# microsoft/ANCE

Hardware: AMD Instinct MI355X
Metric: passages_encoded_per_sec (higher is better)
Workload: dtype f16 pair operands on the fp16 MFMA, f32 accumulate (fp32-grade: <= 2e-5 from the reference's fp32 forward); 1 GPU; MS MARCO passage 8841823 x 768-d, roberta-base rdot_nll FirstP seq_len=128, encode + brute-force IP top-200 (BASELINE configs[1]); encode_block_per_gpu=16384, query_block=32768, layers=12, parallelism=dp1 (corpus rows sharded, top-k all-to-all by query owner + merge)

## Files before the change

ance_amd/csrc/attention.h:

```cpp
#pragma once
#include "common.h"

namespace ance {

struct AttnArgs {
    const _Float16 *qk;
    const _Float16 *vt;
    _Float16 *ctx;
    const int4 *desc;
    int ld_qk, ld_vt, ld_ctx;
    int n_heads;
    int cls_only;
    int q_compact;
};

size_t attention_lds_bytes(int max_seq_len, int n_waves);
int launch_attention_split(const float *qkv, _Float16 *ctx_pair, const int4 *desc, int n_seq, int n_heads, int max_seq_len,
                           int cls_only, hipStream_t stream);
int launch_attention(const AttnArgs &args, int n_seq, int max_seq_len, hipStream_t stream);

}
```

ance_amd/csrc/attention.hip:

```cpp
#include <stdio.h>
#include <stdlib.h>
#include <type_traits>
#include <vector>

#include "common.h"
#include "attention.h"
#include "precise32.h"

namespace ance {
namespace {

constexpr int HD = 64;

__device__ __forceinline__ int kswz(int row, int chunk) { return chunk ^ ((row >> 1) & 7); }

__device__ __forceinline__ void wave_lds_sync() {
    __builtin_amdgcn_fence(__ATOMIC_SEQ_CST, "wavefront");
    __builtin_amdgcn_wave_barrier();
}

__device__ __forceinline__ void attend_qblock(const AttnArgs &A, const _Float16 *Ks, const _Float16 *Vs, const f16x8 (&qf)[4], int s,
                                              int h, int tok0, int T, int Tk, int vld, int qb0, int q_end, int g, int i,
                                              _Float16 *slab) {
    const int nkb = Tk >> 5;
// ... 92 lines not shown
    const int s = dsc.w;
    const int Tk = (T + 31) & ~31;
    const int vld = Tk + 4;
    _Float16 *Ks = reinterpret_cast<_Float16 *>(smem_f);
    _Float16 *Vs = Ks + (size_t)Tk * HD;

    const int tid = threadIdx.x;
    const int w = tid >> 6, l = tid & 63, g = l >> 5, i = l & 31;
    const int H = A.n_heads * HD;
    _Float16 *slab = Vs + (size_t)HD * vld + w * (32 * HD);

    const int q_end = A.cls_only ? 1 : T;
    f16x8 qf[4];
    auto q_row = [&](int r) { return A.q_compact ? (size_t)s : (size_t)(tok0 + min(r, T - 1)); };
    auto q_request = [&](int qb0) {
#pragma unroll
        for (int j = 0; j < 4; ++j) {
            const int row = j * 8 + (l >> 3);
            qf[j] = *reinterpret_cast<const f16x8 *>(A.qk + q_row(qb0 + row) * A.ld_qk + h * HD + (l & 7) * 8);
        }
    };
    auto q_to_fragments = [&]() {
#pragma unroll
        for (int j = 0; j < 4; ++j) {
            const int row = j * 8 + (l >> 3);
            *reinterpret_cast<f16x8 *>(slab + row * HD + kswz(row, l & 7) * 8) = qf[j];
        }
        wave_lds_sync();
#pragma unroll
        for (int sx = 0; sx < 4; ++sx) qf[sx] = *reinterpret_cast<const f16x8 *>(slab + i * HD + kswz(i, 4 * g + sx) * 8);
        wave_lds_sync();
    };
    if (w * 32 < q_end) q_request(w * 32);

    {
        const _Float16 *kbase = A.qk + (size_t)tok0 * A.ld_qk + H + h * HD + (tid & 7) * 8;
        const _Float16 *vbase = A.vt + (size_t)(h * HD) * A.ld_vt + vcol0;
        for (int base = 0; base < Tk; base += 32 * NW) {
            f16x8 kv[4], vv[4];
#pragma unroll
            for (int j = 0; j < 4; ++j) {
                const int row = base + j * (8 * NW) + (tid >> 3);
                const int ev = j * NT + tid, dd = ev / (4 * NW);
                const int key0 = base + (ev - dd * (4 * NW)) * 8;
                kv[j] = f16x8{0, 0, 0, 0, 0, 0, 0, 0};
                vv[j] = f16x8{0, 0, 0, 0, 0, 0, 0, 0};
                if (row < T) kv[j] = *reinterpret_cast<const f16x8 *>(kbase + (size_t)row * A.ld_qk);
                if (key0 < T) vv[j] = *reinterpret_cast<const f16x8 *>(vbase + (size_t)dd * A.ld_vt + key0);
            }
#pragma unroll
            for (int j = 0; j < 4; ++j) {
                const int row = base + j * (8 * NW) + (tid >> 3);
                const int ev = j * NT + tid, dd = ev / (4 * NW);
                const int key0 = base + (ev - dd * (4 * NW)) * 8;
                if (row < Tk) *reinterpret_cast<f16x8 *>(Ks + row * HD + kswz(row, tid & 7) * 8) = kv[j];
                if (key0 < Tk) {
                    if (key0 + 8 > T) {
#pragma unroll
                        for (int e = 0; e < 8; ++e)
                            if (key0 + e >= T) vv[j][e] = (_Float16)0.0f;
                    }
                    _Float16 *dst = Vs + dd * vld + key0;
                    *reinterpret_cast<f16x4 *>(dst) = f16x4{vv[j][0], vv[j][1], vv[j][2], vv[j][3]};
                    *reinterpret_cast<f16x4 *>(dst + 4) = f16x4{vv[j][4], vv[j][5], vv[j][6], vv[j][7]};
                }
            }
        }
    }
    if (w * 32 < q_end) q_to_fragments();
    __syncthreads();

    for (int qb0 = w * 32; qb0 < q_end; qb0 += 32 * NW) {
        if (qb0 != w * 32) {
            q_request(qb0);
            q_to_fragments();
        }
        attend_qblock(A, Ks, Vs, qf, s, h, tok0, T, Tk, vld, qb0, q_end, g, i, slab);
    }
}



constexpr int VS = HD;
__device__ __forceinline__ int vswz(int key, int d) { return d ^ (((key >> 1) & 1) << 5); }
typedef short s16x4_t __attribute__((ext_vector_type(4)));
typedef s16x4_t __attribute__((address_space(3))) lds_s16x4_t;
__device__ __forceinline__ f16x4 lds_read_tr16(const _Float16 *p) {
    const s16x4_t v = __builtin_amdgcn_ds_read_tr16_b64_v4i16((lds_s16x4_t *)(p));
    return __builtin_bit_cast(f16x4, v);
}

__device__ __forceinline__ void permlane32_swap(float &x, float &y) {
    asm volatile("s_nop 1\n\tv_permlane32_swap_b32 %0, %1\n\ts_nop 1" : "+v"(x), "+v"(y));
}

template <int NW>
__global__ void __launch_bounds__(64 * NW, 2) attention_split_kernel(const float *qkv, _Float16 *ctx_pair, const int4 *desc, int n_heads,
                                                                     int cls_only, int kchunk) {
    extern __shared__ __attribute__((aligned(16))) float smem_f[];
    const int u = blockIdx.x / n_heads;
    const int h = blockIdx.x - u * n_heads;
    const int4 dsc = desc[u];
    const int tok0 = dsc.x, T = dsc.y, s = dsc.w;
    const int Tk = (T + 31) & ~31;
    const int kc = Tk < kchunk ? Tk : kchunk;
    _Float16 *Kh = reinterpret_cast<_Float16 *>(smem_f);
    _Float16 *Kl = Kh + (size_t)kc * HD;
    _Float16 *Vh = Kl + (size_t)kc * HD;
    _Float16 *Vl = Vh + (size_t)kc * VS;
    const int tid = threadIdx.x;
    const int w = tid >> 6, l = tid & 63, g = l >> 5, i = l & 31;
    constexpr int NT = 64 * NW;
    const int ld = 3 * n_heads * HD;
    constexpr float SC = 2048.0f, SI = 1.0f / 2048.0f;
    auto stage = [&](int k0, auto unr_tag) {
        constexpr int UNR = decltype(unr_tag)::value;
        for (int e0 = tid; e0 < kc * 8; e0 += UNR * NT) {
            f32x4 kv[UNR][4];
#pragma unroll
            for (int it = 0; it < UNR; ++it) {
                const int e = e0 + it * NT;
                const int kl_ = e >> 3, ch = e & 7, key = k0 + kl_;
#pragma unroll
                for (int q = 0; q < 4; ++q) kv[it][q] = f32x4{0.f, 0.f, 0.f, 0.f};
                if (e < kc * 8 && key < T) {
                    const float *kp = qkv + (size_t)(tok0 + key) * ld + n_heads * HD + h * HD + ch * 8;
                    kv[it][0] = *reinterpret_cast<const f32x4 *>(kp);
                    kv[it][1] = *reinterpret_cast<const f32x4 *>(kp + 4);
                    kv[it][2] = *reinterpret_cast<const f32x4 *>(kp + n_heads * HD);
                    kv[it][3] = *reinterpret_cast<const f32x4 *>(kp + n_heads * HD + 4);
                }
            }
#pragma unroll
            for (int it = 0; it < UNR; ++it) {
                const int e = e0 + it * NT;
                if (e >= kc * 8) break;
                const int kl_ = e >> 3, ch = e & 7;
                const f32x4 k0v = kv[it][0], k1v = kv[it][1], v0 = kv[it][2], v1 = kv[it][3];
                const f16x4 a0 = cvt_f16x4_pinned(k0v), a1 = cvt_f16x4_pinned(k1v), b0 = cvt_f16x4_pinned(v0), b1 = cvt_f16x4_pinned(v1);
                f16x8 kh, kl;
#pragma unroll
                for (int j = 0; j < 4; ++j) {
                    kh[j] = a0[j]; kh[4 + j] = a1[j];
                    kl[j] = (_Float16)((k0v[j] - (float)a0[j]) * SC);
                    kl[4 + j] = (_Float16)((k1v[j] - (float)a1[j]) * SC);
                }
                *reinterpret_cast<f16x8 *>(Kh + kl_ * HD + kswz(kl_, ch) * 8) = kh;
                *reinterpret_cast<f16x8 *>(Kl + kl_ * HD + kswz(kl_, ch) * 8) = kl;
                f16x8 vh, vl;
#pragma unroll
                for (int j = 0; j < 4; ++j) {
                    vh[j] = b0[j]; vh[4 + j] = b1[j];
                    vl[j] = (_Float16)((v0[j] - (float)b0[j]) * SC);
                    vl[4 + j] = (_Float16)((v1[j] - (float)b1[j]) * SC);
                }
                *reinterpret_cast<f16x8 *>(Vh + kl_ * VS + vswz(kl_, ch * 8)) = vh;
                *reinterpret_cast<f16x8 *>(Vl + kl_ * VS + vswz(kl_, ch * 8)) = vl;
            }
        }
    };
    const bool single = Tk <= kc;
    const int q_end = cls_only ? 1 : T;
    const float qscale = 0.125f * 1.44269504088896340736f;
    for (int qp0 = 0; qp0 < q_end; qp0 += 32 * NW) {
        const int qb0 = qp0 + w * 32;
        const bool active = qb0 < q_end;
        f16x8 qh[4], ql[4];
        {
            const float *qp = qkv + (cls_only ? (size_t)s : (size_t)(tok0 + min(qb0 + i, T - 1))) * ld + h * HD + 32 * g;
            f32x4 xq[8];
#pragma unroll
            for (int sx = 0; sx < 8; ++sx) xq[sx] = *reinterpret_cast<const f32x4 *>(qp + sx * 4);
            if (single && qp0 == 0) {
                stage(0, std::integral_constant<int, 4>{});
                __syncthreads();
            }
#pragma unroll
            for (int sx = 0; sx < 4; ++sx) {
                f32x4 x0 = xq[2 * sx], x1 = xq[2 * sx + 1];
                x0 = x0 * qscale;
                x1 = x1 * qscale;
                const f16x4 a0 = cvt_f16x4_pinned(x0), a1 = cvt_f16x4_pinned(x1);
#pragma unroll
                for (int j = 0; j < 4; ++j) {
                    qh[sx][j] = a0[j]; qh[sx][4 + j] = a1[j];
                    ql[sx][j] = (_Float16)((x0[j] - (float)a0[j]) * SC);
                    ql[sx][4 + j] = (_Float16)((x1[j] - (float)a1[j]) * SC);
                }
            }
        }
        float m_run = -INFINITY, l_run = 0.0f;
        f32x16 om0 = {0}, om1 = {0}, oc0 = {0}, oc1 = {0};
        for (int k0 = 0; k0 < Tk; k0 += kc) {
            if (!single) {
                __syncthreads();
                stage(k0, std::integral_constant<int, 1>{});
                __syncthreads();
            }
            if (!active) continue;
            const int nkb = min(kc, Tk - k0) >> 5;
            for (int kb = 0; kb < nkb; ++kb) {
                const int krow = kb * 32 + i;
                const int ksw = (krow >> 1) & 7;
                f32x16 st = {0};
                f16x8 kfh[4];
#pragma unroll
                for (int sx = 0; sx < 4; ++sx) {
                    kfh[sx] = *reinterpret_cast<const f16x8 *>(Kh + krow * HD + (((4 * g + sx) ^ ksw) * 8));
                    const f16x8 kfl = *reinterpret_cast<const f16x8 *>(Kl + krow * HD + (((4 * g + sx) ^ ksw) * 8));
                    st = __builtin_amdgcn_mfma_f32_32x32x16_f16(kfh[sx], ql[sx], st, 0, 0, 0);
                    st = __builtin_amdgcn_mfma_f32_32x32x16_f16(kfl, qh[sx], st, 0, 0, 0);
                }
                st *= SI;
#pragma unroll
                for (int sx = 0; sx < 4; ++sx) st = __builtin_amdgcn_mfma_f32_32x32x16_f16(kfh[sx], qh[sx], st, 0, 0, 0);
                const int key_base = k0 + kb * 32 + 4 * g;
                float bm = -INFINITY;
#pragma unroll
                for (int r = 0; r < 16; ++r) {
                    const int key = key_base + (r & 3) + 8 * (r >> 2);
                    if (k0 + kb * 32 + 32 > T) st[r] = key < T ? st[r] : -INFINITY;
                    bm = fmaxf(bm, st[r]);
                }
                bm = fmaxf(bm, __shfl_xor(bm, 32));
                const float m_new = fmaxf(m_run, bm);
                const float alpha = __builtin_amdgcn_exp2f(m_run - m_new);
                float psum = 0.0f;
                float p[16];
#pragma unroll
                for (int r = 0; r < 16; ++r) {
                    p[r] = __builtin_amdgcn_exp2f(st[r] - m_new);
                    psum += p[r];
                }
                l_run = l_run * alpha + psum;
                m_run = m_new;
                om0 *= alpha; om1 *= alpha; oc0 *= alpha; oc1 *= alpha;
#pragma unroll
                for (int uu = 0; uu < 2; ++uu) {
                    const f16x4 h0 = cvt_f16x4_pinned(f32x4{p[8 * uu], p[8 * uu + 1], p[8 * uu + 2], p[8 * uu + 3]});
                    const f16x4 h1 = cvt_f16x4_pinned(f32x4{p[8 * uu + 4], p[8 * uu + 5], p[8 * uu + 6], p[8 * uu + 7]});
                    f16x8 ph, pl;
#pragma unroll
                    for (int j = 0; j < 4; ++j) {
                        ph[j] = h0[j]; ph[4 + j] = h1[j];
                        pl[j] = (_Float16)((p[8 * uu + j] - (float)h0[j]) * SC);
                        pl[4 + j] = (_Float16)((p[8 * uu + 4 + j] - (float)h1[j]) * SC);
                    }
                    const int kcol = kb * 32 + 16 * uu + 4 * g;
                    auto vfrag = [&](const _Float16 *V, int row) {
                        const int q = l & 15, key = kcol + (q >> 2);
                        const _Float16 *vp = V + key * VS + vswz(key, (row - i) + 16 * ((l >> 4) & 1) + 4 * (q & 3));
                        const f16x4 a = lds_read_tr16(vp), b = lds_read_tr16(vp + 8 * VS);
                        return f16x8{a[0], a[1], a[2], a[3], b[0], b[1], b[2], b[3]};
                    };
                    const f16x8 v0h = vfrag(Vh, i), v1h = vfrag(Vh, i + 32), v0l = vfrag(Vl, i), v1l = vfrag(Vl, i + 32);
                    oc0 = __builtin_amdgcn_mfma_f32_32x32x16_f16(v0h, pl, oc0, 0, 0, 0);
                    oc0 = __builtin_amdgcn_mfma_f32_32x32x16_f16(v0l, ph, oc0, 0, 0, 0);
                    oc1 = __builtin_amdgcn_mfma_f32_32x32x16_f16(v1h, pl, oc1, 0, 0, 0);
                    oc1 = __builtin_amdgcn_mfma_f32_32x32x16_f16(v1l, ph, oc1, 0, 0, 0);
                    om0 = __builtin_amdgcn_mfma_f32_32x32x16_f16(v0h, ph, om0, 0, 0, 0);
                    om1 = __builtin_amdgcn_mfma_f32_32x32x16_f16(v1h, ph, om1, 0, 0, 0);
                }
            }
        }
        if (!active) continue;
        const float l_tot = l_run + __shfl_xor(l_run, 32);
        const float inv = 1.0f / l_tot;
        {
            const bool store = qb0 + i < q_end;
            const size_t orow = cls_only ? (size_t)s : (size_t)(tok0 + min(qb0 + i, T - 1));
            _Float16 *orp = ctx_pair + orow * (size_t)(2 * n_heads * HD);
#pragma unroll
            for (int db = 0; db < 2; ++db) {
                const f32x16 &om = db == 0 ? om0 : om1;
                const f32x16 &oc = db == 0 ? oc0 : oc1;
#pragma unroll
                for (int k2 = 0; k2 < 2; ++k2) {
                    f32x4 va, vb;
#pragma unroll
                    for (int j = 0; j < 4; ++j) {
                        const float xa = __builtin_fmaf(oc[8 * k2 + j], SI, om[8 * k2 + j]) * inv;
                        const float xb = __builtin_fmaf(oc[8 * k2 + 4 + j], SI, om[8 * k2 + 4 + j]) * inv;
                        float sa = xa, sb = xb;
                        permlane32_swap(sa, sb);
                        va[j] = sa;
                        vb[j] = sb;
                    }
                    if (store) {
                        f16x4 ha, ra, hb, rb;
                        pair_split4(va, &ha, &ra);
                        pair_split4(vb, &hb, &rb);
                        const int n = h * HD + db * 32 + 16 * k2 + 8 * g;
                        *reinterpret_cast<f16x8 *>(orp + pair_hi_col(n, n_heads * HD)) = f16x8{ha[0], ha[1], ha[2], ha[3], hb[0], hb[1], hb[2], hb[3]};
                        *reinterpret_cast<f16x8 *>(orp + pair_lo_col(n, n_heads * HD)) = f16x8{ra[0], ra[1], ra[2], ra[3], rb[0], rb[1], rb[2], rb[3]};
                    }
                }
            }
        }
    }
}

}

size_t attention_split_lds_bytes(int max_seq_len) {
    const int Tk = (max_seq_len + 31) & ~31;
    return (size_t)2 * Tk * HD * 2 + (size_t)2 * Tk * VS * 2;
}

int launch_attention_split(const float *qkv, _Float16 *ctx_pair, const int4 *desc, int n_seq, int n_heads, int max_seq_len,
                           int cls_only, hipStream_t st) {
    if (n_seq <= 0) return ANCE_OK;
    const int Tk = (max_seq_len + 31) & ~31;
    const int kchunk = Tk <= 256 ? Tk : 256;
    const size_t lds = attention_split_lds_bytes(kchunk);
    int dev = 0;
    (void)hipGetDevice(&dev);
    static size_t attr_set[64] = {0};
    const bool tracked = dev >= 0 && dev < 64;
    if (!tracked || lds > __atomic_load_n(&attr_set[dev], __ATOMIC_ACQUIRE)) {
        if (hipFuncSetAttribute(reinterpret_cast<const void *>(attention_split_kernel<4>), hipFuncAttributeMaxDynamicSharedMemorySize,
                                (int)lds) != hipSuccess)
            return check_launch("attention_split attr");
        if (tracked) __atomic_store_n(&attr_set[dev], lds, __ATOMIC_RELEASE);
    }
    hipLaunchKernelGGL((attention_split_kernel<4>), dim3((unsigned)n_seq * n_heads), dim3(256), lds, st, qkv, ctx_pair, desc, n_heads,
                       cls_only, kchunk);
    return ANCE_OK;
}

size_t attention_lds_bytes(int max_seq_len, int n_waves) {
    const int Tk = (max_seq_len + 31) & ~31;
    return (size_t)Tk * HD * 2 + (size_t)HD * (Tk + 4) * 2 + (size_t)n_waves * 32 * HD * 2;
}

int launch_attention(const AttnArgs &A, int n_seq, int max_seq_len, hipStream_t st) {
    if (n_seq <= 0) return ANCE_OK;
    const size_t lds = attention_lds_bytes(max_seq_len, 4);
    if (lds > 160 * 1024) {
        set_last_error("attention: sequence too long for LDS");
        return ANCE_E_INVALID;
    }
    int dev = 0;
    (void)hipGetDevice(&dev);
    static size_t attr_set[64] = {0};
    const bool tracked = dev >= 0 && dev < 64;
    if (!tracked || lds > __atomic_load_n(&attr_set[dev], __ATOMIC_ACQUIRE)) {
        if (hipFuncSetAttribute(reinterpret_cast<const void *>(attention_kernel<4>),
                                hipFuncAttributeMaxDynamicSharedMemorySize, (int)lds) != hipSuccess)
            return check_launch("attention attr");
        if (tracked) __atomic_store_n(&attr_set[dev], lds, __ATOMIC_RELEASE);
    }
    hipLaunchKernelGGL((attention_kernel<4>), dim3((unsigned)n_seq * A.n_heads), dim3(256), lds, st, A);
    return ANCE_OK;
}

}

extern "C" int ance_debug_attention(const AnceAttnDebugArgs *a, void *stream) {
    using namespace ance;
    auto refuse = [](const char *why) {
        char buf[160];
        snprintf(buf, sizeof(buf), "ance_debug_attention: invalid argument (%s)", why);
        set_last_error(buf);
        return ANCE_E_INVALID;
    };
    if (!a) return refuse("null args");
    if (a->kind < 0 || a->kind > 2) return refuse("kind");
    if (a->n_heads != 12 && a->n_heads != 16) return refuse("n_heads");
    if (a->n_seq < 1 || a->n_seq > (1 << 20)) return refuse("n_seq");
    if (a->max_seq_len < 1 || a->max_seq_len > 512) return refuse("max_seq_len");
    if (!a->h_desc || !a->d_desc || !a->qk || !a->ctx || (a->kind == 0 && !a->vt)) return refuse("null pointer");
    const int64_t H = 64 * (int64_t)a->n_heads, n = a->n_seq;
    const int64_t desc_bytes = a->kind == 2 ? 4 * (n + 1) : 16 * n;
    if (a->d_desc_bytes < desc_bytes || (uintptr_t)a->d_desc % 16) return refuse("d_desc");
    if ((uintptr_t)a->qk % 16 || (uintptr_t)a->ctx % 16 || (a->kind == 0 && (uintptr_t)a->vt % 16)) return refuse("alignment");
    if (a->qk_rows < 1 || a->ctx_rows < 1) return refuse("rows");
    if (a->kind == 0) {
        if (a->ld_qk % 8 || a->ld_qk < 2 * H || a->ld_vt % 8 || a->ld_vt < 8 || a->ld_ctx % 8 || a->ld_ctx < H) return refuse("stride");
    } else {
        if (a->ld_qk != 3 * H || a->ld_ctx != (a->kind == 1 ? 2 * H : H)) return refuse("stride");
    }
    if (a->kind == 2 && (a->cls_only || a->q_compact)) return refuse("cls_only on kind 2");
    if (a->kind == 1 && a->q_compact != a->cls_only) return refuse("kind 1: q_compact != cls_only");
    if (a->kind == 0 && a->q_compact && !a->cls_only) return refuse("q_compact without cls_only");
    const int32_t *d = a->h_desc;
    if (a->kind == 2) {
        if (d[0] < 0) return refuse("tokens outside the allocation");
        for (int64_t s = 0; s < n; ++s) {
            const int64_t len = (int64_t)d[s + 1] - d[s];
            if (len < 1 || len > a->max_seq_len) return refuse("length");
        }
        if (d[n] > a->qk_rows || d[n] > a->ctx_rows) return refuse("tokens outside the allocation");
    } else {
        std::vector<char> seen((size_t)n, 0);
        const bool compact = a->cls_only && (a->q_compact || a->kind == 1);
        for (int64_t u = 0; u < n; ++u) {
            const int64_t tok0 = d[4 * u], len = d[4 * u + 1], vcol = d[4 * u + 2], s = d[4 * u + 3];
            if (len < 1 || len > a->max_seq_len) return refuse("length");
            if (s < 0 || s >= n || seen[(size_t)s]) return refuse("sequence index");
            seen[(size_t)s] = 1;
            if (tok0 < 0 || tok0 + len > a->qk_rows) return refuse("tokens outside the allocation");
            if (compact && s >= a->qk_rows) return refuse("Q row s past the allocation");
            if (a->cls_only ? s >= a->ctx_rows : tok0 + len > a->ctx_rows) return refuse("output row past the allocation");
            if (a->kind == 0 && (vcol < 0 || vcol % 8 || vcol + ((len + 7) & ~7) > a->ld_vt)) return refuse("V^T columns");
        }
    }
    hipStream_t st = (hipStream_t)stream;
    if (hipMemcpyAsync(a->d_desc, a->h_desc, (size_t)desc_bytes, hipMemcpyHostToDevice, st) != hipSuccess)
        return check_launch("ance_debug_attention: descriptors");
    int rc;
    if (a->kind == 0) {
        AttnArgs A;
        A.qk = (const _Float16 *)a->qk; A.vt = (const _Float16 *)a->vt; A.ctx = (_Float16 *)a->ctx; A.desc = (const int4 *)a->d_desc;
        A.ld_qk = a->ld_qk; A.ld_vt = a->ld_vt; A.ld_ctx = a->ld_ctx; A.n_heads = a->n_heads;
        A.cls_only = a->cls_only ? 1 : 0; A.q_compact = a->q_compact ? 1 : 0;
        rc = launch_attention(A, a->n_seq, a->max_seq_len, st);
    } else if (a->kind == 1) {
        rc = launch_attention_split((const float *)a->qk, (_Float16 *)a->ctx, (const int4 *)a->d_desc, a->n_seq, a->n_heads,
                                    a->max_seq_len, a->cls_only ? 1 : 0, st);
    } else {
        rc = launch_attention32((const float *)a->qk, (float *)a->ctx, (const int *)a->d_desc, a->n_seq, a->n_heads, st);
    }
    return rc ? rc : check_launch("ance_debug_attention");
}
```

ance_amd/csrc/encoder.hip:

```cpp
#include <stdlib.h>
#include <type_traits>
#include <vector>

#include "attention.h"
#include "common.h"
#include "encoder_kernels.h"
#include "encoder_plan.h"
#include "gemm_f16.h"
#include "precise32.h"

namespace ance {
namespace {

template <typename F>
auto with_hidden(int hidden, F &&f) {
    return hidden == 1024 ? f(std::integral_constant<int, 1024>()) : f(std::integral_constant<int, 768>());
}

constexpr int S_CAP_MAX = 8192;
constexpr int FETCH_CHUNK = 262144;
constexpr int MAX_LANES = 2;


bool precise_env() {
// ... 269 lines not shown
}

template <int H>
GemmArgs qk_args(const Rows<FORM_PLANES> &x, int M, float eps, const LayerW &W, int c0, int n, _Float16 *qk) {
    GemmArgs G = folded_args<H>(x, M, eps, W.wqk + (size_t)c0 * H, n, W.bqk + c0, W.cqk + c0);
    G.out16 = qk + c0; G.ldc = 2 * H;
    G.scale = 0.125f * 1.44269504088896340736f; G.scale_cols = c0 == 0 ? H : 0;
    return G;
}
template <int H>
GemmArgs qkv_args(const Rows<FORM_PAIR> &x, int M, float eps, const LayerW &W, int c0, int n, float *qkv, unsigned *faults) {
    GemmArgs G = folded_args<H>(x, M, eps, W.wqkv_s + (size_t)c0 * 2 * H, n, W.bqkv_s + c0, W.cqkv_s + c0, W.sc_s + 4, faults);
    G.out32 = qkv + c0; G.ldc = 3 * H;
    return G;
}

template <int H>
GemmArgs vt_args(const Rows<FORM_PLANES> &x, int Tpad, int T, float eps, const LayerW &W, _Float16 *vt, int ldvt, const int *col_map) {
    GemmArgs G = {};
    G.A = W.wv; G.lda = H; G.B = x.hi; G.tok_lo = x.lo; G.ldb = H; G.M = H; G.N = Tpad; G.K = H;
    G.bias = W.bv; G.csum = W.cv; G.part_in = x.part; G.ln_eps = eps;
    G.out16 = vt; G.ldc = ldvt; G.col_map = col_map; G.n_valid = T;
    return G;
}

template <int H, int FORM>
GemmArgs ffn1_args(const Rows<FORM> &xa, int M, float eps, const LayerW &W, int I, _Float16 *ffn, int n_split, unsigned *faults) {
    constexpr bool P = FORM == FORM_PAIR;
    GemmArgs G = folded_args<H>(xa, M, eps, P ? W.w1_s : W.w1, I, P ? W.b1_s : W.b1, P ? W.c1_s : W.c1, P ? W.sc_s + 6 : nullptr, faults);
    G.out16 = ffn; G.ldc = P ? 2 * I : I; G.n_split = n_split;
    return G;
}

template <int H, int FORM>
GemmArgs resln_args(const _Float16 *A, const _Float16 *B, int K, const float *bias, int M, const Rows<FORM> &res, const float *gamma,
                    const float *beta, float eps, const Rows<FORM> &out, const float *wscale_inv, unsigned *faults) {
    constexpr int w = FORM == FORM_PAIR ? 2 : 1;
    GemmArgs G = {};
    G.A = A; G.lda = w * K; G.B = B; G.ldb = w * K; G.M = M; G.N = H; G.K = K; G.bias = bias; G.ldc = w * H;
    G.res_gamma = gamma; G.res_beta = beta; G.part_in = res.part; G.ln_eps = eps; G.part_out = out.part;
    G.wscale_inv = wscale_inv; G.range_faults = faults;
    if constexpr (FORM == FORM_PAIR) { G.res_hi = res.xp; G.ldr = 2 * H; G.out16 = out.xp; }
    else { G.res_hi = res.hi; G.res_lo = res.lo; G.out16 = out.hi; G.out_lo = out.lo; }
    return G;
}

template <int H>
int forward_split(AnceEncoder *e, const AnceEncoder::Lane &LN, hipStream_t st, const MicroPlan &mb, float *out) {
    constexpr int HP = 2 * H;
    const AnceEncoderDesc &D = e->d;
    const AnceEncoder::Lane::Split &V = LN.sp;
    const int I = D.intermediate, S = mb.S, T = mb.T, Tpad = mb.Tpad;
    {
        ProfScope pe(PC_EMBED, st);
        hipLaunchKernelGGL((embed_kernel<H, FORM_PAIR>), dim3(Tpad / 4), dim3(256), 0, st, LN.tok_id, LN.tok_pos, Tpad, e->word,
                           e->pos, e->type0, D.vocab_size, D.max_position, V.xb, e->faults);
    }
    const bool cls_tail = e->cls_tail;
    const int S_pad = (int)align_up((size_t)S, 256);
    const Rows<FORM_PAIR> cls = V.cls(S_pad, H);
    const int n_split = (I / 256) % 2 == 0 ? 2 : 0;
    for (int li = 0; li < D.n_layers; ++li) {
        const LayerW &W = e->layers[li];
        const bool tail = cls_tail && li == D.n_layers - 1;
        const int Mrows = tail ? S_pad : Tpad;
        const double Mwork = tail ? (double)S : (double)T;
        const float eps_b = li == 0 ? D.ln_eps * (EMB_SCALE * EMB_SCALE) : D.ln_eps;
        const float *const gamma_b = li == 0 ? e->eln_w : e->layers[li - 1].ln2w, *const beta_b = li == 0 ? e->eln_b : e->layers[li - 1].ln2b;
        if (tail) {
            ProfScope ps(PC_LN, st);
            hipLaunchKernelGGL((gather_cls_kernel<H, FORM_PAIR>), dim3(S_pad / 4), dim3(256), 0, st, V.xb, LN.seq_off, S, S_pad, cls);
        }
        {
            ProfScope ps(PC_GEMM_QK, st, tail ? 2.0 * T * (2.0 * H) * H + 2.0 * S * (double)H * H : 2.0 * T * (3.0 * H) * H);
            const int c0 = tail ? H : 0;
            int rc = launch_gemm_f16(EPI_S_QKV, qkv_args<H>(V.xb, Tpad, eps_b, W, c0, 3 * H - c0, V.qkv, e->faults), st, H);
            if (tail && !rc) rc = launch_gemm_f16(EPI_S_QKV, qkv_args<H>(cls, S_pad, eps_b, W, 0, H, V.qkv, e->faults), st, H);
            if (rc) return rc;
        }
        {
            ProfScope ps(PC_ATTN, st);
            if (tail && S_pad > S)
                (void)hipMemsetAsync(V.ctx + (size_t)S * HP, 0, (size_t)(S_pad - S) * HP * sizeof(_Float16), st);
            if (int rc = launch_attention_split(V.qkv, V.ctx, LN.desc, S, D.n_heads, mb.maxlen, tail ? 1 : 0, st)) return rc;
        }
        if (ProfScope ps(PC_GEMM_OUT, st, 2.0 * Mwork * (double)H * H);
            int rc = launch_gemm_f16(EPI_S_RESLN, resln_args<H>(V.ctx, W.wo_s, H, W.bo, Mrows, tail ? cls : V.xb, gamma_b, beta_b, eps_b,
                                                                V.xa, W.sc_s + 5, e->faults), st, H))
            return rc;
        if (ProfScope ps(PC_GEMM_FFN1, st, 2.0 * Mwork * (double)I * H);
            int rc = launch_gemm_f16(EPI_S_GELU, ffn1_args<H>(V.xa, Mrows, D.ln_eps, W, I, V.ffn, n_split, e->faults), st, H))
            return rc;
        if (ProfScope ps(PC_GEMM_FFN2, st, 2.0 * Mwork * (double)I * H);
            int rc = launch_gemm_f16(EPI_S_RESLN, resln_args<H>(V.ffn, W.w2_s, I, W.b2, Mrows, V.xa, W.ln1w, W.ln1b, D.ln_eps, V.xb,
                                                                W.sc_s + 7, e->faults), st, H))
            return rc;
    }
    encoder_output<H>(e, LN, st, mb, out, V.xb, cls_tail ? 1 : 0);
    return ANCE_OK;
}

template <int H>
int forward_fp16(AnceEncoder *e, const AnceEncoder::Lane &LN, hipStream_t st, const MicroPlan &mb, float *out) {
    const AnceEncoderDesc &D = e->d;
    const AnceEncoder::Lane::Fp16 &V = LN.f16;
    const int I = D.intermediate, S = mb.S, T = mb.T, Tpad = mb.Tpad;
    {
        ProfScope pe(PC_EMBED, st);
        hipLaunchKernelGGL((embed_kernel<H, FORM_PLANES>), dim3(Tpad / 4), dim3(256), 0, st, LN.tok_id, LN.tok_pos, Tpad, e->word,
                           e->pos, e->type0, D.vocab_size, D.max_position, V.xb, (unsigned *)nullptr);
    }
    const bool cls_tail = e->cls_tail;
    const int S_pad = (int)align_up((size_t)S, 256);
    const Rows<FORM_PLANES> cls = V.cls(S_pad, H);
    const int n_split = (I / 256) % 2 == 0 ? 2 : 0;
    for (int li = 0; li < D.n_layers; ++li) {
        const LayerW &W = e->layers[li];
        const bool tail = cls_tail && li == D.n_layers - 1;
        const int Mrows = tail ? S_pad : Tpad;
        const double Mwork = tail ? (double)S : (double)T;
        const float *const gamma_b = li == 0 ? e->eln_w : e->layers[li - 1].ln2w, *const beta_b = li == 0 ? e->eln_b : e->layers[li - 1].ln2b;
        if (tail) {
            ProfScope ps(PC_LN, st);
            hipLaunchKernelGGL((gather_cls_kernel<H, FORM_PLANES>), dim3(S_pad / 4), dim3(256), 0, st, V.xb, LN.seq_off, S, S_pad, cls);
        }
        {
            ProfScope ps(PC_GEMM_QK, st, tail ? 2.0 * T * (double)H * H + 2.0 * S * (double)H * H : 2.0 * T * (2.0 * H) * H);
            const int c0 = tail ? H : 0;
            int rc = launch_gemm_f16(EPI_QK_F, qk_args<H>(V.xb, Tpad, D.ln_eps, W, c0, 2 * H - c0, V.qk), st, H);
            if (tail && !rc) rc = launch_gemm_f16(EPI_QK_F, qk_args<H>(cls, S_pad, D.ln_eps, W, 0, H, V.qk), st, H);
            if (rc) return rc;
        }
        if (ProfScope ps(PC_GEMM_VT, st, 2.0 * T * (double)H * H);
            int rc = launch_gemm_f16(EPI_VT_F, vt_args<H>(V.xb, Tpad, T, D.ln_eps, W, V.vt, mb.ldvt, LN.tok_vtcol), st, H))
            return rc;
        AttnArgs A;
        A.qk = V.qk; A.vt = V.vt; A.ctx = V.ctx; A.desc = LN.desc;
        A.ld_qk = 2 * H; A.ld_vt = mb.ldvt; A.ld_ctx = H; A.n_heads = D.n_heads; A.cls_only = tail ? 1 : 0; A.q_compact = tail ? 1 : 0;
        if (ProfScope ps(PC_ATTN, st, 0.0); int rc = launch_attention(A, S, mb.maxlen, st)) return rc;
        if (ProfScope ps(PC_GEMM_OUT, st, 2.0 * Mwork * (double)H * H);
            int rc = launch_gemm_f16(EPI_RESLN, resln_args<H>(V.ctx, W.wo, H, W.bo, Mrows, tail ? cls : V.xb, gamma_b, beta_b, D.ln_eps,
                                                              V.xa, nullptr, nullptr), st, H))
            return rc;
        if (ProfScope ps(PC_GEMM_FFN1, st, 2.0 * Mwork * (double)I * H);
            int rc = launch_gemm_f16(EPI_GELU_F, ffn1_args<H>(V.xa, Mrows, D.ln_eps, W, I, V.ffn, n_split, nullptr), st, H))
            return rc;
        if (ProfScope ps(PC_GEMM_FFN2, st, 2.0 * Mwork * (double)I * H);
            int rc = launch_gemm_f16(EPI_RESLN, resln_args<H>(V.ffn, W.w2, I, W.b2, Mrows, V.xa, W.ln1w, W.ln1b, D.ln_eps, V.xb,
                                                              nullptr, nullptr), st, H))
            return rc;
    }
    encoder_output<H>(e, LN, st, mb, out, V.xb, cls_tail ? 1 : 0);
    return ANCE_OK;
}

struct LaneFork {
    AnceEncoder *e;
    hipStream_t caller_st;
    bool forked = false;
    void fork() {
        (void)hipEventRecord(e->ev_fork, caller_st);
        for (int ln = 0; ln < e->n_lanes; ++ln) (void)hipStreamWaitEvent(e->side[ln], e->ev_fork, 0);
        forked = true;
    }
    void join_lanes() {
        for (int ln = 0; forked && ln < e->n_lanes; ++ln) {
            (void)hipEventRecord(e->ev_join[ln], e->side[ln]);
// ... 300 lines not shown
```

ance_amd/csrc/encoder_plan.h:

```cpp
#pragma once
#include "common.h"

namespace ance {
namespace {

__host__ __device__ inline int clamp_len(int full, int L) { return full < 0 ? 0 : (full > L ? L : full); }
__host__ __device__ inline int chunk_len(int full, int c, int Lc) {
    const int lc = full - c * Lc;
    return lc < 0 ? 0 : (lc > Lc ? Lc : lc);
}
__host__ __device__ inline int eff_len(int lc) { return lc > 0 ? lc : 1; }
__host__ __device__ inline int vt_width(int eff) { return (eff + 7) & ~7; }
__host__ __device__ inline int len_bucket(int eff) {
    const int b = (eff + 31) >> 5;
    return b > 4 ? 3 : b - 1;
}

struct MicroPlan {
    int S, T, V;
    int maxlen;
    int Tpad, ldvt;
    int64_t next;
};
inline MicroPlan plan_micro_batch(const int32_t *hl, int64_t first, int64_t end, int n_chunks, int L, int Lc, int scap, int tcap,
                                  int vcap, bool seed) {
    MicroPlan p = {0, 0, 0, 1, 0, 0, first};
    while (p.next < end && p.S < scap) {
        const int64_t rec = p.next / n_chunks;
        const int eff = eff_len(chunk_len(clamp_len(hl[rec], L), (int)(p.next - rec * n_chunks), Lc));
        if (p.T + eff > tcap || p.V + vt_width(eff) > vcap - 256) break;
        p.T += eff; p.V += vt_width(eff); ++p.S; ++p.next;
        if (eff > p.maxlen) p.maxlen = eff;
    }
    p.Tpad = (int)align_up((size_t)p.T, 256);
    p.ldvt = (int)align_up((size_t)p.V + (seed ? 8 : 0), 256);
    return p;
}


__device__ __forceinline__ int record_len(const int32_t *ids_or_rec, int64_t ld, const int32_t *lens, int64_t rec, int L) {
    int full;
    if (lens) full = lens[rec];
    else full = (int)__builtin_bswap32((uint32_t)ids_or_rec[rec * ld]);
    return clamp_len(full, L);
}

__global__ void fetch_lens_kernel(const int32_t *base, int64_t ld, const int32_t *lens, int64_t r0, int n, int L, int32_t *out) {
    const int i = blockIdx.x * blockDim.x + threadIdx.x;
    if (i < n) out[i] = record_len(base, ld, lens, r0 + i, L);
}

struct PlanArgs {
    const int32_t *base;
    int64_t ld;
    const int32_t *lens;
    int hdr;
    int64_t g0;
    int S;
    int L, n_chunks, Lc;
    int pad_id, arch;
    int T, Tpad;
    int vt_spare;
    int *seq_off, *seq_vtcol, *seq_len;
    int *tok_id, *tok_pos, *tok_vtcol;
    int4 *desc;
    unsigned *faults;
};

__global__ void __launch_bounds__(256) seed_count_kernel(const PlanArgs P) {
    const int s = blockIdx.x * 4 + (threadIdx.x >> 6);
    const int l = threadIdx.x & 63;
    if (s >= P.S) return;
    const int64_t rec = P.g0 + s;
    const int full = record_len(P.base, P.ld, P.lens, rec, P.L);
    const int32_t *src = P.base + rec * P.ld + P.hdr;
    int cnt = 0;
    for (int j0 = 0; j0 < full; j0 += 64) {
        const int j = j0 + l;
        cnt += __popcll(__ballot(j < full && src[j] != P.pad_id));
    }
    if (l == 0) {
        P.seq_len[s] = cnt;
        if (full == 0 || src[0] == P.pad_id) atomicAdd(P.faults + 1, 1u);
    }
}

__global__ void __launch_bounds__(1024) plan_kernel(const PlanArgs P) {
    __shared__ int s_tot[1024], s_tot8[1024];
    __shared__ unsigned long long s_bk[1024];
    const int tid = threadIdx.x;
    const int per = (P.S + 1023) / 1024;
    const int b0 = tid * per;
    int sum = 0, sum8 = 0;
    unsigned long long bk = 0;
    for (int j = 0; j < per; ++j) {
        const int s = b0 + j;
        if (s < P.S) {
            int lc;
            if (P.arch == ANCE_ARCH_SEED) {
                lc = P.seq_len[s];
            } else {
                const int64_t gs = P.g0 + s;
                const int64_t rec = gs / P.n_chunks;
                const int c = (int)(gs - rec * P.n_chunks);
                lc = chunk_len(record_len(P.base, P.ld, P.lens, rec, P.L), c, P.Lc);
                P.seq_len[s] = lc;
            }
            const int eff = eff_len(lc);
            sum += eff;
            sum8 += vt_width(eff);
            bk += 1ull << (16 * len_bucket(eff));
        }
    }
    s_tot[tid] = sum;
    s_tot8[tid] = sum8;
    s_bk[tid] = bk;
// ... 104 lines not shown
```

Baseline: 32980 passages/s.

## Pack two short sequences per attention workgroup and use buffer loads for K/V staging

Sequences of at most 64 tokens, which come after the long ones in length-bucketed order, are now paired: each workgroup splits into two half-groups with their own LDS slice, so short passages no longer leave most waves idle. K/V staging switches to raw buffer loads with bounds-checked descriptors and a different element-to-thread mapping that writes f16x4 halves, and Q loads are issued before staging to overlap latency. This adds branching, relies on the planner's n_long counting matching the bucket order, and can increase LDS per block for the paired case.

```diff
diff --git a/ance_amd/csrc/attention.h b/ance_amd/csrc/attention.h
--- a/ance_amd/csrc/attention.h
+++ b/ance_amd/csrc/attention.h
@@ -15,7 +15,7 @@
 };
 
 size_t attention_lds_bytes(int max_seq_len, int n_waves);
-int launch_attention_split(const float *qkv, _Float16 *ctx_pair, const int4 *desc, int n_seq, int n_heads, int max_seq_len,
+int launch_attention_split(const float *qkv, _Float16 *ctx_pair, const int4 *desc, int n_seq, int n_long, int n_heads, int max_seq_len,
                            int cls_only, hipStream_t stream);
 int launch_attention(const AttnArgs &args, int n_seq, int max_seq_len, hipStream_t stream);
 
diff --git a/ance_amd/csrc/attention.hip b/ance_amd/csrc/attention.hip
--- a/ance_amd/csrc/attention.hip
+++ b/ance_amd/csrc/attention.hip
@@ -198,6 +198,7 @@
 
 
 constexpr int VS = HD;
+constexpr int PAIR_T = 64;
 __device__ __forceinline__ int vswz(int key, int d) { return d ^ (((key >> 1) & 1) << 5); }
 typedef short s16x4_t __attribute__((ext_vector_type(4)));
 typedef s16x4_t __attribute__((address_space(3))) lds_s16x4_t;
@@ -212,85 +213,94 @@
 
 template <int NW>
 __global__ void __launch_bounds__(64 * NW, 2) attention_split_kernel(const float *qkv, _Float16 *ctx_pair, const int4 *desc, int n_heads,
-                                                                     int cls_only, int kchunk) {
+                                                                     int cls_only, int kchunk, int n_long, int n_seq) {
     extern __shared__ __attribute__((aligned(16))) float smem_f[];
     const int u = blockIdx.x / n_heads;
     const int h = blockIdx.x - u * n_heads;
-    const int4 dsc = desc[u];
+    const bool paired = u >= n_long;
+    const int side = paired ? __builtin_amdgcn_readfirstlane((int)threadIdx.x / (32 * NW)) : 0;
+    const int nw_sub = paired ? NW / 2 : NW;
+    const int du = paired ? n_long + 2 * (u - n_long) + side : u;
+    int4 dsc = desc[du < n_seq ? du : n_seq - 1];
+    if (du >= n_seq || (paired && (dsc.y > PAIR_T || dsc.y > kchunk))) dsc = make_int4(0, 0, 0, 0);
     const int tok0 = dsc.x, T = dsc.y, s = dsc.w;
     const int Tk = (T + 31) & ~31;
     const int kc = Tk < kchunk ? Tk : kchunk;
-    _Float16 *Kh = reinterpret_cast<_Float16 *>(smem_f);
+    _Float16 *Kh = reinterpret_cast<_Float16 *>(smem_f) + (size_t)side * 4 * (kchunk < PAIR_T ? kchunk : PAIR_T) * HD;
     _Float16 *Kl = Kh + (size_t)kc * HD;
     _Float16 *Vh = Kl + (size_t)kc * HD;
     _Float16 *Vl = Vh + (size_t)kc * VS;
-    const int tid = threadIdx.x;
+    const int tid = (int)threadIdx.x - side * (32 * NW);
     const int w = tid >> 6, l = tid & 63, g = l >> 5, i = l & 31;
-    constexpr int NT = 64 * NW;
+    const int NT = 64 * nw_sub;
     const int ld = 3 * n_heads * HD;
     constexpr float SC = 2048.0f, SI = 1.0f / 2048.0f;
-    auto stage = [&](int k0, auto unr_tag) {
+    const int Hb = n_heads * HD * 4;
+    const auto panel = __builtin_amdgcn_make_buffer_rsrc(
+        const_cast<float *>(qkv + (size_t)tok0 * ld + n_heads * HD + h * HD), 0, T > 0 ? (T - 1) * ld * 4 + Hb + HD * 4 : 0, 0x00020000);
+    auto panel_load = [&](int byte_off) __attribute__((always_inline)) {
+        return __builtin_bit_cast(f32x4, __builtin_amdgcn_raw_buffer_load_b128(panel, byte_off, 0, 0));
+    };
+    auto stage = [&](int k0, auto unr_tag) __attribute__((always_inline)) {
         constexpr int UNR = decltype(unr_tag)::value;
         for (int e0 = tid; e0 < kc * 8; e0 += UNR * NT) {
             f32x4 kv[UNR][4];
 #pragma unroll
             for (int it = 0; it < UNR; ++it) {
                 const int e = e0 + it * NT;
-                const int kl_ = e >> 3, ch = e & 7, key = k0 + kl_;
-#pragma unroll
-                for (int q = 0; q < 4; ++q) kv[it][q] = f32x4{0.f, 0.f, 0.f, 0.f};
-                if (e < kc * 8 && key < T) {
-                    const float *kp = qkv + (size_t)(tok0 + key) * ld + n_heads * HD + h * HD + ch * 8;
-                    kv[it][0] = *reinterpret_cast<const f32x4 *>(kp);
-                    kv[it][1] = *reinterpret_cast<const f32x4 *>(kp + 4);
-                    kv[it][2] = *reinterpret_cast<const f32x4 *>(kp + n_heads * HD);
-                    kv[it][3] = *reinterpret_cast<const f32x4 *>(kp + n_heads * HD + 4);
-                }
+                const int ka = ((e >> 6) << 3) + ((e & 63) >> 4), c = e & 15;
+                const int bo = ((k0 + ka) * ld + c * 4) * 4;
+                kv[it][0] = panel_load(bo);
+                kv[it][2] = panel_load(bo + Hb);
+                kv[it][1] = panel_load(bo + 16 * ld);
+                kv[it][3] = panel_load(bo + 16 * ld + Hb);
             }
 #pragma unroll
             for (int it = 0; it < UNR; ++it) {
                 const int e = e0 + it * NT;
                 if (e >= kc * 8) break;
-                const int kl_ = e >> 3, ch = e & 7;
-                const f32x4 k0v = kv[it][0], k1v = kv[it][1], v0 = kv[it][2], v1 = kv[it][3];
-                const f16x4 a0 = cvt_f16x4_pinned(k0v), a1 = cvt_f16x4_pinned(k1v), b0 = cvt_f16x4_pinned(v0), b1 = cvt_f16x4_pinned(v1);
-                f16x8 kh, kl;
-#pragma unroll
-                for (int j = 0; j < 4; ++j) {
-                    kh[j] = a0[j]; kh[4 + j] = a1[j];
-                    kl[j] = (_Float16)((k0v[j] - (float)a0[j]) * SC);
-                    kl[4 + j] = (_Float16)((k1v[j] - (float)a1[j]) * SC);
-                }
-                *reinterpret_cast<f16x8 *>(Kh + kl_ * HD + kswz(kl_, ch) * 8) = kh;
-                *reinterpret_cast<f16x8 *>(Kl + kl_ * HD + kswz(kl_, ch) * 8) = kl;
-                f16x8 vh, vl;
-#pragma unroll
-                for (int j = 0; j < 4; ++j) {
-                    vh[j] = b0[j]; vh[4 + j] = b1[j];
-                    vl[j] = (_Float16)((v0[j] - (float)b0[j]) * SC);
-                    vl[4 + j] = (_Float16)((v1[j] - (float)b1[j]) * SC);
-                }
-                *reinterpret_cast<f16x8 *>(Vh + kl_ * VS + vswz(kl_, ch * 8)) = vh;
-                *reinterpret_cast<f16x8 *>(Vl + kl_ * VS + vswz(kl_, ch * 8)) = vl;
+                const int ka = ((e >> 6) << 3) + ((e & 63) >> 4), c = e & 15;
+#pragma unroll
+                for (int hk = 0; hk < 2; ++hk) {
+                    const int kl_ = ka + 4 * hk;
+                    const f32x4 kx = kv[it][hk], vx = kv[it][2 + hk];
+                    const f16x4 a = cvt_f16x4_pinned(kx), b = cvt_f16x4_pinned(vx);
+                    f16x4 kl, vl;
+#pragma unroll
+                    for (int j = 0; j < 4; ++j) {
+                        kl[j] = (_Float16)((kx[j] - (float)a[j]) * SC);
+                        vl[j] = (_Float16)((vx[j] - (float)b[j]) * SC);
+                    }
+                    const int ko = kl_ * HD + kswz(kl_, c >> 1) * 8 + (c & 1) * 4, vo = kl_ * VS + vswz(kl_, c * 4);
+                    *reinterpret_cast<f16x4 *>(Kh + ko) = a;
+                    *reinterpret_cast<f16x4 *>(Kl + ko) = kl;
+                    *reinterpret_cast<f16x4 *>(Vh + vo) = b;
+                    *reinterpret_cast<f16x4 *>(Vl + vo) = vl;
+                }
             }
         }
     };
     const bool single = Tk <= kc;
-    const int q_end = cls_only ? 1 : T;
+    const int q_end = cls_only ? min(T, 1) : T;
     const float qscale = 0.125f * 1.44269504088896340736f;
-    for (int qp0 = 0; qp0 < q_end; qp0 += 32 * NW) {
+    f32x4 xq[8];
+    auto q_request = [&](int qp0) __attribute__((always_inline)) {
+        const float *qp = qkv + (cls_only ? (size_t)s : (size_t)(tok0 + max(min(qp0 + w * 32 + i, T - 1), 0))) * ld + h * HD + 32 * g;
+#pragma unroll
+        for (int sx = 0; sx < 8; ++sx) xq[sx] = *reinterpret_cast<const f32x4 *>(qp + sx * 4);
+    };
+    q_request(0);
+    if (single) {
+        stage(0, std::integral_constant<int, 4>{});
+        __syncthreads();
+    }
+    int qp0 = 0;
+    do {
         const int qb0 = qp0 + w * 32;
         const bool active = qb0 < q_end;
         f16x8 qh[4], ql[4];
         {
-            const float *qp = qkv + (cls_only ? (size_t)s : (size_t)(tok0 + min(qb0 + i, T - 1))) * ld + h * HD + 32 * g;
-            f32x4 xq[8];
-#pragma unroll
-            for (int sx = 0; sx < 8; ++sx) xq[sx] = *reinterpret_cast<const f32x4 *>(qp + sx * 4);
-            if (single && qp0 == 0) {
-                stage(0, std::integral_constant<int, 4>{});
-                __syncthreads();
-            }
+            if (qp0 != 0) q_request(qp0);
 #pragma unroll
             for (int sx = 0; sx < 4; ++sx) {
                 f32x4 x0 = xq[2 * sx], x1 = xq[2 * sx + 1];
@@ -413,7 +423,7 @@
                 }
             }
         }
-    }
+    } while ((qp0 += 32 * nw_sub) < q_end);
 }
 
 }
@@ -423,12 +433,18 @@
     return (size_t)2 * Tk * HD * 2 + (size_t)2 * Tk * VS * 2;
 }
 
-int launch_attention_split(const float *qkv, _Float16 *ctx_pair, const int4 *desc, int n_seq, int n_heads, int max_seq_len,
+int launch_attention_split(const float *qkv, _Float16 *ctx_pair, const int4 *desc, int n_seq, int n_long, int n_heads, int max_seq_len,
                            int cls_only, hipStream_t st) {
     if (n_seq <= 0) return ANCE_OK;
+    if (n_long < 0 || n_long > n_seq) {
+        set_last_error("attention_split: n_long outside [0, n_seq]");
+        return ANCE_E_INVALID;
+    }
     const int Tk = (max_seq_len + 31) & ~31;
     const int kchunk = Tk <= 256 ? Tk : 256;
-    const size_t lds = attention_split_lds_bytes(kchunk);
+    const size_t lds_one = attention_split_lds_bytes(kchunk), lds_two = 2 * attention_split_lds_bytes(kchunk < PAIR_T ? kchunk : PAIR_T);
+    const size_t lds = n_long < n_seq && lds_two > lds_one ? lds_two : lds_one;
+    const int n_wg = n_long + (n_seq - n_long + 1) / 2;
     int dev = 0;
     (void)hipGetDevice(&dev);
     static size_t attr_set[64] = {0};
@@ -439,8 +455,8 @@
             return check_launch("attention_split attr");
         if (tracked) __atomic_store_n(&attr_set[dev], lds, __ATOMIC_RELEASE);
     }
-    hipLaunchKernelGGL((attention_split_kernel<4>), dim3((unsigned)n_seq * n_heads), dim3(256), lds, st, qkv, ctx_pair, desc, n_heads,
-                       cls_only, kchunk);
+    hipLaunchKernelGGL((attention_split_kernel<4>), dim3((unsigned)n_wg * n_heads), dim3(256), lds, st, qkv, ctx_pair, desc, n_heads,
+                       cls_only, kchunk, n_long, n_seq);
     return ANCE_OK;
 }
 
@@ -532,8 +548,16 @@
         A.cls_only = a->cls_only ? 1 : 0; A.q_compact = a->q_compact ? 1 : 0;
         rc = launch_attention(A, a->n_seq, a->max_seq_len, st);
     } else if (a->kind == 1) {
-        rc = launch_attention_split((const float *)a->qk, (_Float16 *)a->ctx, (const int4 *)a->d_desc, a->n_seq, a->n_heads,
-                                    a->max_seq_len, a->cls_only ? 1 : 0, st);
+        int n_long = 0;
+        bool longs_first = true;
+        for (int64_t u = 0; u < n; ++u) {
+            if (d[4 * u + 1] > PAIR_T) {
+                if (n_long != u) longs_first = false;
+                ++n_long;
+            }
+        }
+        rc = launch_attention_split((const float *)a->qk, (_Float16 *)a->ctx, (const int4 *)a->d_desc, a->n_seq,
+                                    longs_first ? n_long : a->n_seq, a->n_heads, a->max_seq_len, a->cls_only ? 1 : 0, st);
     } else {
         rc = launch_attention32((const float *)a->qk, (float *)a->ctx, (const int *)a->d_desc, a->n_seq, a->n_heads, st);
     }
diff --git a/ance_amd/csrc/encoder.hip b/ance_amd/csrc/encoder.hip
--- a/ance_amd/csrc/encoder.hip
+++ b/ance_amd/csrc/encoder.hip
@@ -375,7 +375,7 @@
             ProfScope ps(PC_ATTN, st);
             if (tail && S_pad > S)
                 (void)hipMemsetAsync(V.ctx + (size_t)S * HP, 0, (size_t)(S_pad - S) * HP * sizeof(_Float16), st);
-            if (int rc = launch_attention_split(V.qkv, V.ctx, LN.desc, S, D.n_heads, mb.maxlen, tail ? 1 : 0, st)) return rc;
+            if (int rc = launch_attention_split(V.qkv, V.ctx, LN.desc, S, mb.n_long, D.n_heads, mb.maxlen, tail ? 1 : 0, st)) return rc;
         }
         if (ProfScope ps(PC_GEMM_OUT, st, 2.0 * Mwork * (double)H * H);
             int rc = launch_gemm_f16(EPI_S_RESLN, resln_args<H>(V.ctx, W.wo_s, H, W.bo, Mrows, tail ? cls : V.xb, gamma_b, beta_b, eps_b,
diff --git a/ance_amd/csrc/encoder_plan.h b/ance_amd/csrc/encoder_plan.h
--- a/ance_amd/csrc/encoder_plan.h
+++ b/ance_amd/csrc/encoder_plan.h
@@ -21,17 +21,20 @@
     int maxlen;
     int Tpad, ldvt;
     int64_t next;
+    int n_long;
 };
 inline MicroPlan plan_micro_batch(const int32_t *hl, int64_t first, int64_t end, int n_chunks, int L, int Lc, int scap, int tcap,
                                   int vcap, bool seed) {
-    MicroPlan p = {0, 0, 0, 1, 0, 0, first};
+    MicroPlan p = {0, 0, 0, 1, 0, 0, first, 0};
     while (p.next < end && p.S < scap) {
         const int64_t rec = p.next / n_chunks;
         const int eff = eff_len(chunk_len(clamp_len(hl[rec], L), (int)(p.next - rec * n_chunks), Lc));
         if (p.T + eff > tcap || p.V + vt_width(eff) > vcap - 256) break;
         p.T += eff; p.V += vt_width(eff); ++p.S; ++p.next;
         if (eff > p.maxlen) p.maxlen = eff;
-    }
+        if (len_bucket(eff) >= 2) ++p.n_long;
+    }
+    if (seed) p.n_long = p.S;
     p.Tpad = (int)align_up((size_t)p.T, 256);
     p.ldvt = (int)align_up((size_t)p.V + (seed ? 8 : 0), 256);
     return p;
```

New measurement: 33130 passages/s, median of 6. No clear change (+0.4%).
